# angela000/DQNFlappyBird

Measured on NVIDIA B200. Metric: env frames/sec (step+render+preproc), higher is better.
Workload: dtype u8

## Files before the change

dqnflappybird_b200/csrc/fb_common.cuh:

```cuda
#pragma once
#include <cuda_runtime.h>
#include <stdint.h>
#include <string>

#include "../../include/flappy_b200.h"

void fb_set_error(const std::string &msg);

#define FB_CUDA_OK(expr)                                                                      \
    do {                                                                                      \
        cudaError_t _e = (expr);                                                              \
        if (_e != cudaSuccess) {                                                              \
            fb_set_error(std::string(#expr) + ": " + cudaGetErrorString(_e));                 \
            return FB_ERR_CUDA;                                                               \
        }                                                                                     \
    } while (0)

#define FB_REQUIRE(cond, msg)                                                                 \
    do {                                                                                      \
        if (!(cond)) { fb_set_error(std::string(msg)); return FB_ERR_INVALID; }               \
    } while (0)

constexpr int kScreenW = 288, kScreenH = 512;
constexpr int kBirdW = 34, kBirdH = 24;
constexpr int kPipeW = 52, kPipeH = 320;
constexpr int kBaseW = 336, kBaseH = 112;
constexpr int kPlayerX = 57;
constexpr int kInitY = 244;
constexpr int kBaseYDraw = 404;
constexpr int kGroundY = 380;
constexpr int kBaseShift = kBaseW - kScreenW;
constexpr int kGapSize = 100;
constexpr int kMaxY = 379;

constexpr int kObs = FB_OBS;
constexpr int kBaseJ = 63;
constexpr int kBirdRows = 9;

struct __align__(16) EnvState {
    int16_t y;
    int8_t vel;
    uint8_t pidx;
    uint8_t loop;
    uint8_t phase;
    int8_t basex;
    uint8_t npipes;
    int16_t px[3];
    uint8_t gap[3];
    uint8_t pad0;
    int16_t pad1;
    int32_t score;
    uint32_t draws;
    uint32_t pad2;
};
static_assert(sizeof(EnvState) == 32, "EnvState must be 32 bytes");

struct ObsTables {
    unsigned long long pipeObs[54][5][8];
    unsigned char birdObs[3][kMaxY + 1][kBirdRows + 3];
    unsigned char birdJ0[kMaxY + 1 + 4];
    short sx[kObs];
};

static_assert(sizeof(ObsTables) % 16 == 0, "ObsTables is copied with 16-byte loads");

struct HitTables {
    unsigned long long birdRow[3][kBirdH];
    unsigned long long pipeRowLo[kPipeH];
    unsigned long long pipeRowUp[kPipeH];
};
static_assert(sizeof(HitTables) % 16 == 0, "HitTables is copied with 16-byte loads");

struct ExactTables {
    unsigned long long birdRow[3][kBirdH];
    unsigned long long pipeRowLo[kPipeH];
    unsigned long long pipeRowUp[kPipeH];
    uint32_t birdPix[3][kBirdW][kBirdH];
    uint32_t pipeLo[kPipeW][kPipeH];
    uint32_t pipeUp[kPipeW][kPipeH];
    uint32_t basePix[kBaseW][kBaseH];
    int sx[kObs], a0[kObs], a1[kObs];
    int sy[kObs], b0[kObs], b1[kObs];
};

struct FbTables {
    ObsTables *obs_dev;
    ExactTables *exact_dev;
    int device;
    bool loaded;
};
const FbTables &fb_tables();
const ObsTables *fb_host_obs_tables();
const ExactTables *fb_host_exact_tables();

__host__ __device__ inline void philox4x32_10(uint32_t c0, uint32_t c1, uint32_t c2, uint32_t c3, uint32_t k0,
                                              uint32_t k1, uint32_t out[4]) {
#pragma unroll
    for (int r = 0; r < 10; r++) {
#ifdef __CUDA_ARCH__
        uint32_t h0 = __umulhi(0xD2511F53u, c0), l0 = 0xD2511F53u * c0;
        uint32_t h1 = __umulhi(0xCD9E8D57u, c2), l1 = 0xCD9E8D57u * c2;
#else
        uint64_t p0 = (uint64_t)0xD2511F53u * c0, p1 = (uint64_t)0xCD9E8D57u * c2;
        uint32_t h0 = (uint32_t)(p0 >> 32), l0 = (uint32_t)p0, h1 = (uint32_t)(p1 >> 32), l1 = (uint32_t)p1;
#endif
        uint32_t n0 = h1 ^ c1 ^ k0, n2 = h0 ^ c3 ^ k1;
        c0 = n0; c1 = l1; c2 = n2; c3 = l0;
        k0 += 0x9E3779B9u; k1 += 0xBB67AE85u;
    }
    out[0] = c0; out[1] = c1; out[2] = c2; out[3] = c3;
}

__host__ __device__ inline uint32_t stream_word(uint64_t seed, uint32_t purpose, uint64_t env, uint32_t n) {
    uint32_t o[4];
    philox4x32_10(n >> 2, purpose, (uint32_t)env, (uint32_t)(env >> 32), (uint32_t)seed, (uint32_t)(seed >> 32), o);
    return o[n & 3];
}

__host__ __device__ inline int obs_pixel_gt1(uint32_t p00, uint32_t p01, uint32_t p10, uint32_t p11, int a0, int a1,
                                             int b0, int b1) {
    int v[3];
#pragma unroll
    for (int c = 0; c < 3; c++) {
        int s = 8 * c;
        int h0 = (int)((p00 >> s) & 255) * b0 + (int)((p01 >> s) & 255) * b1;
        int h1 = (int)((p10 >> s) & 255) * b0 + (int)((p11 >> s) & 255) * b1;
        v[c] = (((a0 * (h0 >> 4)) >> 16) + ((a1 * (h1 >> 4)) >> 16) + 2) >> 2;
    }
    int g = (3735 * v[0] + 19235 * v[1] + 9798 * v[2] + (1 << 14)) >> 15;
    return g > 1;
}
```

dqnflappybird_b200/csrc/fb_debug.cu:

```cuda
#include <stddef.h>
#include <string.h>

#include "fb_env_logic.cuh"

extern "C" int fb_debug_host_step(int32_t *state16, int action, const uint8_t *gaps, int gaps_len, uint64_t seed,
                                  uint64_t env_id, float *reward, uint8_t *terminal, int32_t *score) {
    const ExactTables *ex = fb_host_exact_tables();
    if (!ex) { fb_set_error("fb_debug_host_step: load the assets first"); return FB_ERR_ASSETS; }
    FB_REQUIRE(state16 && reward && terminal && score, "fb_debug_host_step: NULL argument");
    if (action != 0 && action != 1) { fb_set_error("Multiple input actions!"); return FB_ERR_ACTION; }
    EnvState s;
    memset(&s, 0, sizeof(s));
    if (!ints_to_state(state16, s)) { fb_set_error("fb_debug_host_step: state outside the reachable range"); return FB_ERR_STATE; }
    GapSource g{gaps, gaps_len, seed, env_id};
    env_step(s, action, g, ex, *reward, *terminal, *score);
    state_to_ints(s, state16);
    return FB_OK;
}

extern "C" int fb_debug_host_reset(int32_t *state16, const uint8_t *gaps, int gaps_len, uint64_t seed, uint64_t env_id) {
    FB_REQUIRE(state16 != nullptr, "fb_debug_host_reset: NULL argument");
    EnvState s;
    memset(&s, 0, sizeof(s));
    GapSource g{gaps, gaps_len, seed, env_id};
    env_reset(s, g);
    state_to_ints(s, state16);
    return FB_OK;
}

extern "C" int fb_debug_host_obs(const int32_t *state16, int mode, uint8_t *out) {
    const ObsTables *T = fb_host_obs_tables();
    const ExactTables *ex = fb_host_exact_tables();
    if (!T || !ex) { fb_set_error("fb_debug_host_obs: load the assets first"); return FB_ERR_ASSETS; }
    EnvState s;
    memset(&s, 0, sizeof(s));
    if (!ints_to_state(state16, s)) { fb_set_error("fb_debug_host_obs: state outside the reachable range"); return FB_ERR_STATE; }
    DrawList d = make_draw_list(s);
    if (mode == 1) {
        for (int i = 0; i < kObs; i++)
            for (int j = 0; j < kObs; j++) out[i * kObs + j] = exact_obs_bit(ex, d, s.basex, true, i, j) ? 255 : 0;
        return FB_OK;
    }
    const int j0 = T->birdJ0[d.y];
    for (int i = 0; i < kObs; i++) {
        unsigned long long m = obs_row_mask(*T, d, i);
        int r = i - 16;
        if ((d.np_mixed & 16) && r >= 0 && r < kBirdRows) {
            unsigned byte = 0;
            for (int b = 0; b < 8; b++)
                if (j0 + b < kBaseJ && exact_obs_bit(ex, d, 0, false, i, j0 + b)) byte |= 1u << b;
            m = obs_row_fix(m, byte, j0);
        }
        for (int j = 0; j < kObs; j++) out[i * kObs + j] = (j >= 64 || ((m >> j) & 1)) ? 255 : 0;
    }
    return FB_OK;
}

extern "C" int fb_debug_host_mixed(const int32_t *state16) {
    EnvState s;
    memset(&s, 0, sizeof(s));
    if (!ints_to_state(state16, s)) return -1;
    return (make_draw_list(s).np_mixed & 16) ? 1 : 0;
}

extern "C" int fb_debug_step_sampling_layout(int32_t *out, int capacity) {
    const int32_t v[] = {(int32_t)sizeof(fb_step_sampling),
                         (int32_t)offsetof(fb_step_sampling, replay), (int32_t)offsetof(fb_step_sampling, ring_dev),
                         (int32_t)offsetof(fb_step_sampling, act_dev), (int32_t)offsetof(fb_step_sampling, rew_dev),
                         (int32_t)offsetof(fb_step_sampling, term_dev), (int32_t)offsetof(fb_step_sampling, t),
                         (int32_t)offsetof(fb_step_sampling, batch), (int32_t)offsetof(fb_step_sampling, setsize),
                         (int32_t)offsetof(fb_step_sampling, seed), (int32_t)offsetof(fb_step_sampling, idx_out_dev),
                         (int32_t)offsetof(fb_step_sampling, frames_out_dev), (int32_t)offsetof(fb_step_sampling, act_out_dev),
                         (int32_t)offsetof(fb_step_sampling, rew_out_dev), (int32_t)offsetof(fb_step_sampling, term_out_dev),
                         (int32_t)offsetof(fb_step_sampling, env_out_dev), (int32_t)offsetof(fb_step_sampling, k_out_dev),
                         (int32_t)offsetof(fb_step_sampling, prioritized), (int32_t)offsetof(fb_step_sampling, per_mode),
                         (int32_t)offsetof(fb_step_sampling, beta), (int32_t)offsetof(fb_step_sampling, tree_idx_out_dev),
                         (int32_t)offsetof(fb_step_sampling, is_weights_out_dev), (int32_t)offsetof(fb_step_sampling, prio_out_dev),
                         (int32_t)offsetof(fb_step_sampling, is_weights_f32_out_dev)};
    const int n = (int)(sizeof(v) / sizeof(v[0]));
    FB_REQUIRE(out != nullptr && capacity >= n, "fb_debug_step_sampling_layout: buffer too small");
    for (int i = 0; i < n; i++) out[i] = v[i];
    return n;
}

__global__ void __launch_bounds__(256) write_probe_kernel(uint8_t *dst, int n_chunks, long long stride_bytes, int mode) {
    extern __shared__ __align__(128) uint8_t stage_all[];
    const int warp = threadIdx.x >> 5, lane = threadIdx.x & 31;
    uint8_t *stage = stage_all + warp * 6400;
    const long long W = (long long)gridDim.x * 8, w = (long long)blockIdx.x * 8 + warp;
    const int lo = (int)((long long)n_chunks * w / W), hi = (int)((long long)n_chunks * (w + 1) / W);
    if (mode == 1) {
        for (int i = lane; i < 400; i += 32) reinterpret_cast<uint4 *>(stage)[i] = make_uint4(i, lane, 0xFFFFFFFFu, 0);
        asm volatile("fence.proxy.async.shared::cta;" ::: "memory");
        __syncwarp();
    }
    for (int k = lo; k < hi; k++) {
        uint8_t *out = dst + (long long)k * stride_bytes;
        if (mode == 0) {
            const uint4 v = make_uint4(k, lane, 0xFFFFFFFFu, 0);
#pragma unroll
            for (int it = 0; it < 13; it++) { int c = lane + 32 * it; if (c < 400) __stcs(reinterpret_cast<uint4 *>(out) + c, v); }
        } else if (lane == 0) {
            asm volatile("cp.async.bulk.wait_group.read 0;" ::: "memory");
            asm volatile("cp.async.bulk.global.shared::cta.bulk_group [%0], [%1], 6400;" ::"l"(reinterpret_cast<uint64_t>(out)),
                         "r"((uint32_t)__cvta_generic_to_shared(stage)) : "memory");
            asm volatile("cp.async.bulk.commit_group;" ::: "memory");
        }
    }
    if (mode == 1 && lane == 0) asm volatile("cp.async.bulk.wait_group 0;" ::: "memory");
}

extern "C" int fb_debug_write_probe(uint8_t *dst_dev, int n_chunks, long long stride_bytes, int mode, int ctas, void *stream) {
    FB_REQUIRE(dst_dev && n_chunks > 0 && stride_bytes >= 6400 && (mode == 0 || mode == 1) && ctas > 0, "fb_debug_write_probe: bad argument");
    FB_CUDA_OK(cudaFuncSetAttribute(write_probe_kernel, cudaFuncAttributeMaxDynamicSharedMemorySize, 8 * 6400));
    write_probe_kernel<<<ctas, 256, 8 * 6400, (cudaStream_t)stream>>>(dst_dev, n_chunks, stride_bytes, mode);
    FB_CUDA_OK(cudaGetLastError());
    return FB_OK;
}
```

dqnflappybird_b200/csrc/fb_env.cu:

```cuda
#include <stdlib.h>

#include <new>

#include "fb_env_logic.cuh"

struct fb_env {
    int n;
    uint64_t seed, first_id;
    EnvState *state;
    const uint8_t *gaps;
    int gaps_len;
    int *err_flag;
    uint8_t *stage_act[2];
    float *stage_rew[2];
    uint8_t *stage_term[2];
    int32_t *stage_score[2];
    cudaStream_t s_in, s_out;
    cudaEvent_t ev_in[2], ev_step[2], ev_out[2];
    unsigned long long submitted, waited;
    int num_sms;
    int step_slots;
};

struct StepArgs {
    EnvState *state;
    int n;
    uint64_t seed, first_id;
    const uint8_t *gaps;
    int gaps_len;
    const uint8_t *actions;
    uint64_t act_seed;
    uint32_t first_step, flap_threshold;
    uint8_t *actions_out;
    uint8_t *ring;
    int ring_len, ring_slot;
    float *reward;
    uint8_t *terminal;
    int32_t *score;
    int n_steps;
    int draw_only;
    int *err_flag;
    const ObsTables *obs_tab;
    const ExactTables *ex;
};

__device__ __forceinline__ uint32_t expand4(uint32_t nib) {
    return ((nib * 0x00204081u) & 0x01010101u) * 255u;
}

struct RowConst { int sx[3], tab[3]; };

struct __align__(16) DrawWords {
    int px[3];
    int flags;
    int goff[3];
    int bird;
};
__device__ __forceinline__ DrawWords to_words(const ObsTables &T, const DrawList &d) {
    DrawWords w;
    const int np = d.np_mixed & 15;
#pragma unroll
    for (int k = 0; k < 3; k++) { w.px[k] = k < np ? (int)d.px[k] : 9999; w.goff[k] = (int)d.gap[k] * 8; }
    w.flags = ((d.np_mixed & 16) ? 1 : 0) | ((int)T.birdJ0[d.y] << 1) | ((int)d.y << 8) | ((int)d.pidx << 20) | (np << 24);
    w.bird = ((int)d.pidx * (kMaxY + 1) + (int)d.y) * (kBirdRows + 3);
    return w;
}

constexpr int kChunks = kObs * 5;

__device__ __forceinline__ void render_env(const ObsTables &T, const uint2 *lut8, const ExactTables *ex, const DrawWords w,
                                           const RowConst &rc, unsigned short *m16, unsigned long long *fixrows, uint8_t *out, int lane) {
    const int j0 = (w.flags >> 1) & 127;
    const unsigned char *pipe_bytes = reinterpret_cast<const unsigned char *>(&T.pipeObs[0][0][0]);
    const unsigned char *bird_bytes = reinterpret_cast<const unsigned char *>(&T.birdObs[0][0][0]) + w.bird;
    unsigned long long m[3];
#pragma unroll
    for (int it = 0; it < 3; it++) {
        unsigned long long v = 1ull << 63;
#pragma unroll
        for (int k = 0; k < 3; k++) {
            const unsigned c = (unsigned)(rc.sx[it] - w.px[k] + 1);
            if (c < 54u) v |= *reinterpret_cast<const unsigned long long *>(pipe_bytes + c * 320u + rc.tab[it] + w.goff[k]);
        }
        m[it] = v;
    }
    if (lane >= 16 && lane < 16 + kBirdRows) m[0] |= (unsigned long long)bird_bytes[lane - 16] << j0;
    if (w.flags & 1) {
        DrawList d;
        d.y = (int16_t)((w.flags >> 8) & 4095); d.pidx = (uint8_t)((w.flags >> 20) & 3); d.np_mixed = (uint8_t)(((w.flags >> 24) & 15) | 16);
#pragma unroll
        for (int k = 0; k < 3; k++) { d.px[k] = (int16_t)(w.px[k] == 9999 ? 0 : w.px[k]); d.gap[k] = (uint8_t)(w.goff[k] >> 3); d.pad[k] = 0; }
        if (lane >= 16 && lane < 16 + kBirdRows) fixrows[lane - 16] = m[0];
        __syncwarp();
#pragma unroll 1
        for (int q = 0; q < 3; q++) {
            int idx = q * 32 + lane, r = idx >> 3, j = j0 + (idx & 7);
            int bit = 0;
            if (r < kBirdRows && j < kBaseJ) bit = exact_obs_bit(ex, d, 0, false, 16 + r, j);
            unsigned bal = __ballot_sync(0xFFFFFFFFu, bit);
            int rr = 4 * q + lane;
            if (lane < 4 && rr < kBirdRows) fixrows[rr] = obs_row_fix(fixrows[rr], (bal >> (8 * lane)) & 0xFFu, j0);
        }
        __syncwarp();
        if (lane >= 16 && lane < 16 + kBirdRows) m[0] = fixrows[lane - 16];
    }
#pragma unroll
    for (int it = 0; it < 3; it++) {
        const int i = lane + 32 * it;
        if (i < kObs) {
            unsigned short *row = m16 + 5 * i;
            row[0] = (unsigned short)m[it]; row[1] = (unsigned short)(m[it] >> 16);
            row[2] = (unsigned short)(m[it] >> 32); row[3] = (unsigned short)(m[it] >> 48);
        }
    }
    __syncwarp();
    const unsigned short *mine = m16 + lane;
    uint4 *dst = reinterpret_cast<uint4 *>(out) + lane;
#pragma unroll
    for (int it = 0; it < 13; it++) {
        if (it < 12 || lane < kChunks - 32 * 12) {
            const uint32_t bits = mine[32 * it];
            const uint2 a = lut8[bits & 255u], b = lut8[bits >> 8];
            __stcs(dst + 32 * it, make_uint4(a.x, a.y, b.x, b.y));
        }
    }
    __syncwarp();
}

constexpr int kStepThreads = 256, kStepWarps = kStepThreads / 32;

__global__ void __launch_bounds__(kStepThreads, 4) env_step_kernel(const StepArgs a) {
    extern __shared__ __align__(16) unsigned char t_raw[];
    ObsTables &T = *reinterpret_cast<ObsTables *>(t_raw);
    __shared__ __align__(16) HitTables H;
    __shared__ DrawWords dw[kStepWarps][32];
    __shared__ __align__(16) unsigned short m16[kStepWarps][kChunks + 8];
    __shared__ unsigned long long fixrows[kStepWarps][kBirdRows + 1];
    __shared__ uint2 lut8[256];
    const int tid = threadIdx.x, warp = tid >> 5, lane = tid & 31;
    asm volatile("griddepcontrol.launch_dependents;");
    lut8[tid] = make_uint2(expand4(tid & 15u), expand4(tid >> 4));

    {
        const uint4 *srcH = reinterpret_cast<const uint4 *>(a.ex);
        uint4 *dstH = reinterpret_cast<uint4 *>(&H);
        for (int k = tid; k < (int)(sizeof(HitTables) / 16); k += kStepThreads) dstH[k] = __ldg(srcH + k);
    }
    if (a.ring) {
        const uint4 *src = reinterpret_cast<const uint4 *>(a.obs_tab);
        uint4 *dstT = reinterpret_cast<uint4 *>(&T);
        for (int k = tid; k < (int)(sizeof(ObsTables) / 16); k += kStepThreads) dstT[k] = __ldg(src + k);
    }
    __syncthreads();
    asm volatile("griddepcontrol.wait;" ::: "memory");

    RowConst rc;
#pragma unroll
    for (int it = 0; it < 3; it++) {
        const int i = min(lane + 32 * it, kObs - 1);
        rc.sx[it] = T.sx[i]; rc.tab[it] = (i - 5 * ((i * 205) >> 10)) * 64;
    }
    for (int i = lane; i < kObs; i += 32) m16[warp][5 * i + 4] = 0xFFFFu;
    __syncwarp();
    const long long W = (long long)gridDim.x * kStepWarps, w = (long long)blockIdx.x * kStepWarps + warp;
    const int lo = (int)((long long)a.n * w / W), hi = (int)((long long)a.n * (w + 1) / W);
    for (int base = lo; base < hi; base += 32) {
        const int e_mine = base + lane;
        const bool have = e_mine < hi;
        const int n_here = min(32, hi - base);
        EnvState s;
        GapSource gs;
        if (have) {
            const uint4 *sp = reinterpret_cast<const uint4 *>(a.state + e_mine);
            uint4 v0 = sp[0], v1 = sp[1];
            *reinterpret_cast<uint4 *>(&s) = v0;
            *(reinterpret_cast<uint4 *>(&s) + 1) = v1;
            gs.script = a.gaps ? a.gaps + (size_t)e_mine * a.gaps_len : nullptr;
            gs.script_len = a.gaps_len;
            gs.seed = a.seed; gs.env_id = a.first_id + (uint64_t)e_mine;
        }
        for (int step = 0; step < a.n_steps; step++) {
            if (have && a.draw_only) dw[warp][lane] = to_words(T, make_draw_list(s));
            if (have && !a.draw_only) {
                int act;
                const size_t o = (size_t)step * a.n + e_mine;
                if (a.actions) {
                    act = a.actions[o];
                    if (act > 1) { atomicOr(a.err_flag, 1); act = 0; }
                } else {
                    act = stream_word(a.act_seed, 1u, gs.env_id, a.first_step + (uint32_t)step) < a.flap_threshold ? 1 : 0;
                    if (a.actions_out) a.actions_out[o] = (uint8_t)act;
                }
                float rew; uint8_t term; int32_t sc;
                env_step(s, act, gs, &H, rew, term, sc);
                if (a.reward) a.reward[o] = rew;
                if (a.terminal) a.terminal[o] = term;
                if (a.score) a.score[o] = sc;
                if (a.ring) dw[warp][lane] = to_words(T, make_draw_list(s));
            }
            if (a.ring) {
                const int slot = (a.ring_slot + step) % a.ring_len;
                __syncwarp();
                for (int e = 0; e < n_here; e++) {
                    uint8_t *out = a.ring + ((size_t)(base + e) * a.ring_len + slot) * (size_t)FB_FRAME_BYTES;
                    render_env(T, lut8, a.ex, dw[warp][e], rc, m16[warp], fixrows[warp], out, lane);
                }
                __syncwarp();
            }
        }
        if (have) {
            uint4 *sp = reinterpret_cast<uint4 *>(a.state + e_mine);
            sp[0] = *reinterpret_cast<uint4 *>(&s);
            sp[1] = *(reinterpret_cast<uint4 *>(&s) + 1);
        }
    }
}


__global__ void env_reset_kernel(EnvState *state, int n, uint64_t seed, uint64_t first_id, const uint8_t *gaps, int gaps_len) {
    int e = blockIdx.x * blockDim.x + threadIdx.x;
    if (e >= n) return;
    EnvState s;
    memset(&s, 0, sizeof(s));
    GapSource gs{gaps ? gaps + (size_t)e * gaps_len : nullptr, gaps_len, seed, first_id + (uint64_t)e};
    env_reset(s, gs);
    state[e] = s;
}

__global__ void env_export_kernel(const EnvState *state, int n, int32_t *out) {
    int e = blockIdx.x * blockDim.x + threadIdx.x;
    if (e >= n) return;
    EnvState s = state[e];
    state_to_ints(s, out + (size_t)e * FB_STATE_INTS);
}

__global__ void env_import_kernel(EnvState *state, int n, const int32_t *in, int *err_flag) {
    int e = blockIdx.x * blockDim.x + threadIdx.x;
    if (e >= n) return;
    EnvState s;
    if (!ints_to_state(in + (size_t)e * FB_STATE_INTS, s)) { atomicOr(err_flag, 2); return; }
    state[e] = s;
}

__global__ void env_obs_exact_kernel(const EnvState *state, int n, const ExactTables *ex, uint8_t *obs) {
    int e = blockIdx.x;
    if (e >= n) return;
    __shared__ DrawList d;
    __shared__ int basex;
    if (threadIdx.x == 0) { EnvState s = state[e]; d = make_draw_list(s); basex = s.basex; }
    __syncthreads();
    for (int p = threadIdx.x; p < kObs * kObs; p += blockDim.x) {
        int i = p / kObs, j = p - i * kObs;
        obs[(size_t)e * FB_FRAME_BYTES + p] = exact_obs_bit(ex, d, basex, true, i, j) ? 255 : 0;
    }
}

__global__ void env_render_full_kernel(const EnvState *state, int first, int n, const ExactTables *ex, uint8_t *rgb) {
    int e = blockIdx.y;
    if (e >= n) return;
    __shared__ DrawList d;
    __shared__ int basex;
    if (threadIdx.x == 0) { EnvState s = state[first + e]; d = make_draw_list(s); basex = s.basex; }
    __syncthreads();
    int p = blockIdx.x * blockDim.x + threadIdx.x;
    if (p >= kScreenW * kScreenH) return;
    int X = p / kScreenH, Y = p - X * kScreenH;
    uint32_t c = scene_rgb(ex, d, basex, true, X, Y);
    uint8_t *o = rgb + ((size_t)e * kScreenW * kScreenH + p) * 3;
    o[0] = c & 255; o[1] = (c >> 8) & 255; o[2] = (c >> 16) & 255;
}


extern "C" int fb_env_create(int n_envs, uint64_t seed, uint64_t first_env_id, fb_env **out) {
    FB_REQUIRE(out != nullptr, "fb_env_create: out is NULL");
    FB_REQUIRE(n_envs > 0, "fb_env_create: n_envs must be positive");
    if (!fb_tables().loaded) { fb_set_error("fb_env_create: call fb_assets_load first"); return FB_ERR_ASSETS; }
    fb_env *e = new (std::nothrow) fb_env();
    FB_REQUIRE(e != nullptr, "fb_env_create: out of host memory");
    e->n = n_envs; e->seed = seed; e->first_id = first_env_id; e->gaps = nullptr; e->gaps_len = 0;
    int dev = 0;
    FB_CUDA_OK(cudaGetDevice(&dev));
    FB_CUDA_OK(cudaDeviceGetAttribute(&e->num_sms, cudaDevAttrMultiProcessorCount, dev));
    FB_CUDA_OK(cudaMalloc(&e->state, sizeof(EnvState) * (size_t)n_envs));
    FB_CUDA_OK(cudaMalloc(&e->err_flag, sizeof(int)));
    FB_CUDA_OK(cudaMemset(e->err_flag, 0, sizeof(int)));
    for (int k = 0; k < 2; k++) {
        FB_CUDA_OK(cudaMalloc(&e->stage_act[k], (size_t)n_envs));
        FB_CUDA_OK(cudaMalloc(&e->stage_rew[k], sizeof(float) * (size_t)n_envs));
        FB_CUDA_OK(cudaMalloc(&e->stage_term[k], (size_t)n_envs));
        FB_CUDA_OK(cudaMalloc(&e->stage_score[k], sizeof(int32_t) * (size_t)n_envs));
        FB_CUDA_OK(cudaEventCreateWithFlags(&e->ev_in[k], cudaEventDisableTiming));
        FB_CUDA_OK(cudaEventCreateWithFlags(&e->ev_step[k], cudaEventDisableTiming));
        FB_CUDA_OK(cudaEventCreateWithFlags(&e->ev_out[k], cudaEventDisableTiming));
    }
    FB_CUDA_OK(cudaStreamCreateWithFlags(&e->s_in, cudaStreamNonBlocking));
    FB_CUDA_OK(cudaStreamCreateWithFlags(&e->s_out, cudaStreamNonBlocking));
    e->submitted = e->waited = 0;
    e->step_slots = 0;
    *out = e;
    return fb_env_reset(e, nullptr);
}

extern "C" int fb_env_destroy(fb_env *e) {
    if (!e) return FB_OK;
    cudaFree(e->state); cudaFree(e->err_flag);
    for (int k = 0; k < 2; k++) {
        cudaFree(e->stage_act[k]); cudaFree(e->stage_rew[k]); cudaFree(e->stage_term[k]); cudaFree(e->stage_score[k]);
        if (e->ev_in[k]) cudaEventDestroy(e->ev_in[k]);
        if (e->ev_step[k]) cudaEventDestroy(e->ev_step[k]);
        if (e->ev_out[k]) cudaEventDestroy(e->ev_out[k]);
    }
    if (e->s_in) cudaStreamDestroy(e->s_in);
    if (e->s_out) cudaStreamDestroy(e->s_out);
    delete e;
    return FB_OK;
}

extern "C" int fb_env_num_envs(const fb_env *e) { return e ? e->n : 0; }

extern "C" int fb_env_set_gap_replay(fb_env *e, const uint8_t *gaps_dev, int per_env_len) {
    FB_REQUIRE(e != nullptr, "fb_env_set_gap_replay: env is NULL");
    FB_REQUIRE(gaps_dev == nullptr || per_env_len > 0, "fb_env_set_gap_replay: per_env_len must be positive");
    e->gaps = gaps_dev; e->gaps_len = gaps_dev ? per_env_len : 0;
    return FB_OK;
}

extern "C" int fb_env_reset(fb_env *e, void *stream) {
    FB_REQUIRE(e != nullptr, "fb_env_reset: env is NULL");
    env_reset_kernel<<<(e->n + 255) / 256, 256, 0, (cudaStream_t)stream>>>(e->state, e->n, e->seed, e->first_id, e->gaps, e->gaps_len);
    FB_CUDA_OK(cudaGetLastError());
    return FB_OK;
}

static int launch_step(fb_env *e, StepArgs &a, cudaStream_t st, bool early = true) {
    a.state = e->state; a.n = e->n; a.seed = e->seed; a.first_id = e->first_id;
    a.gaps = e->gaps; a.gaps_len = e->gaps_len; a.err_flag = e->err_flag;
    a.obs_tab = fb_tables().obs_dev; a.ex = fb_tables().exact_dev;
    if (e->step_slots == 0) {
        FB_CUDA_OK(cudaFuncSetAttribute(env_step_kernel, cudaFuncAttributeMaxDynamicSharedMemorySize, (int)sizeof(ObsTables)));
        int per_sm = 0;
        FB_CUDA_OK(cudaOccupancyMaxActiveBlocksPerMultiprocessor(&per_sm, env_step_kernel, kStepThreads, sizeof(ObsTables)));
        FB_REQUIRE(per_sm >= 1, "env_step_kernel does not fit an SM");
        e->step_slots = per_sm * e->num_sms;
    }
    static int oversub = 0;
    if (oversub == 0) { const char *v = getenv("FB_ENV_OVERSUB"); oversub = (v && v[0] >= '1' && v[0] <= '8') ? v[0] - '0' : 1; }
    long long warps = (long long)e->step_slots * kStepWarps * oversub;
    if (warps > e->n) warps = e->n;
    const int grid = (int)((warps + kStepWarps - 1) / kStepWarps);
    cudaLaunchConfig_t cfg{};
    cfg.gridDim = dim3(grid); cfg.blockDim = dim3(kStepThreads); cfg.dynamicSmemBytes = sizeof(ObsTables); cfg.stream = st;
    cudaLaunchAttribute at[1];
    at[0].id = cudaLaunchAttributeProgrammaticStreamSerialization;
    static int pdl = -1;
    if (pdl < 0) { const char *v = getenv("FB_ENV_PDL"); pdl = (v && v[0] == '0') ? 0 : 1; }
    at[0].val.programmaticStreamSerializationAllowed = pdl && early ? 1 : 0;
    cfg.attrs = at; cfg.numAttrs = 1;
    FB_CUDA_OK(cudaLaunchKernelEx(&cfg, env_step_kernel, (const StepArgs)a));
    return FB_OK;
}

static int check_ring(const fb_env *e, const uint8_t *ring, int ring_len, int ring_slot, int n_steps) {
    FB_REQUIRE(e != nullptr, "fb_env_step: env is NULL");
    FB_REQUIRE(n_steps > 0, "fb_env_step: n_steps must be positive");
    if (ring) {
        FB_REQUIRE(ring_len > 0 && ring_slot >= 0 && ring_slot < ring_len, "fb_env_step: ring_slot outside the ring");
        FB_REQUIRE((reinterpret_cast<uintptr_t>(ring) & 15) == 0, "fb_env_step: obs ring must be 16-byte aligned");
    }
    return FB_OK;
}

extern "C" int fb_env_step(fb_env *e, int n_steps, const uint8_t *actions_dev, uint8_t *obs_ring_dev, int ring_len,
                           int ring_slot, float *reward_dev, uint8_t *terminal_dev, int32_t *score_dev, void *stream) {
    int rc = check_ring(e, obs_ring_dev, ring_len, ring_slot, n_steps);
    if (rc) return rc;
    FB_REQUIRE(actions_dev != nullptr, "fb_env_step: actions_dev is NULL");
    StepArgs a{};
    a.actions = actions_dev; a.ring = obs_ring_dev; a.ring_len = ring_len; a.ring_slot = ring_slot;
    a.reward = reward_dev; a.terminal = terminal_dev; a.score = score_dev; a.n_steps = n_steps;
    return launch_step(e, a, (cudaStream_t)stream);
}

extern "C" int fb_env_draw(fb_env *e, uint8_t *obs_ring_dev, int ring_len, int ring_slot, void *stream) {
    int rc = check_ring(e, obs_ring_dev, ring_len, ring_slot, 1);
    if (rc) return rc;
    FB_REQUIRE(obs_ring_dev != nullptr, "fb_env_draw: obs_ring_dev is NULL");
    StepArgs a{};
    a.ring = obs_ring_dev; a.ring_len = ring_len; a.ring_slot = ring_slot; a.n_steps = 1; a.draw_only = 1;
    return launch_step(e, a, (cudaStream_t)stream);
}

extern "C" int fb_env_step_random(fb_env *e, int n_steps, uint64_t action_seed, uint32_t first_step, uint32_t flap_threshold,
                                  uint8_t *actions_out_dev, uint8_t *obs_ring_dev, int ring_len, int ring_slot,
                                  float *reward_dev, uint8_t *terminal_dev, int32_t *score_dev, void *stream) {
    int rc = check_ring(e, obs_ring_dev, ring_len, ring_slot, n_steps);
    if (rc) return rc;
    StepArgs a{};
    a.actions = nullptr; a.act_seed = action_seed; a.first_step = first_step; a.flap_threshold = flap_threshold;
    a.actions_out = actions_out_dev; a.ring = obs_ring_dev; a.ring_len = ring_len; a.ring_slot = ring_slot;
    a.reward = reward_dev; a.terminal = terminal_dev; a.score = score_dev; a.n_steps = n_steps;
    return launch_step(e, a, (cudaStream_t)stream);
}

static int host_submit(fb_env *e, const uint8_t *actions_host, uint8_t *obs_ring_dev, int ring_len, int ring_slot,
                       float *reward_host, uint8_t *terminal_host, int32_t *score_host, void *stream, bool split) {
    int rc = check_ring(e, obs_ring_dev, ring_len, ring_slot, 1);
    if (rc) return rc;
    FB_REQUIRE(actions_host != nullptr, "fb_env_step_host: actions_host is NULL");
    FB_REQUIRE(e->submitted - e->waited < 2, "fb_env_step_host_submit: two steps are already in flight; call fb_env_step_host_wait");
    cudaStream_t st = (cudaStream_t)stream;
    {
        const int n = e->n;
        int k = 0;
        unsigned long long bad = 0;
        for (; k + 8 <= n; k += 8) { unsigned long long w; memcpy(&w, actions_host + k, 8); bad |= w & 0xFEFEFEFEFEFEFEFEull; }
        for (; k < n; k++) bad |= (unsigned long long)(actions_host[k] & 0xFE);
        if (bad) { fb_set_error("Multiple input actions!"); return FB_ERR_ACTION; }
    }
    const int sl = (int)(e->submitted & 1);
    FB_CUDA_OK(cudaMemcpyAsync(e->stage_act[sl], actions_host, (size_t)e->n, cudaMemcpyHostToDevice, e->s_in));
    FB_CUDA_OK(cudaEventRecord(e->ev_in[sl], e->s_in));
    FB_CUDA_OK(cudaStreamWaitEvent(st, e->ev_in[sl], 0));
    StepArgs a{};
    a.actions = e->stage_act[sl]; a.ring = obs_ring_dev; a.ring_len = ring_len; a.ring_slot = ring_slot;
    a.reward = e->stage_rew[sl]; a.terminal = e->stage_term[sl]; a.score = e->stage_score[sl]; a.n_steps = 1;
    split = split && obs_ring_dev != nullptr;
    if (split) a.ring = nullptr;
    rc = launch_step(e, a, st, false);
    if (rc) return rc;
    FB_CUDA_OK(cudaEventRecord(e->ev_step[sl], st));
    if (split) {
        StepArgs d{};
        d.ring = obs_ring_dev; d.ring_len = ring_len; d.ring_slot = ring_slot; d.n_steps = 1; d.draw_only = 1;
        rc = launch_step(e, d, st);
        if (rc) return rc;
        FB_CUDA_OK(cudaEventRecord(e->ev_in[sl], st));
    }
    FB_CUDA_OK(cudaStreamWaitEvent(e->s_out, e->ev_step[sl], 0));
    if (reward_host) FB_CUDA_OK(cudaMemcpyAsync(reward_host, e->stage_rew[sl], sizeof(float) * (size_t)e->n, cudaMemcpyDeviceToHost, e->s_out));
    if (terminal_host) FB_CUDA_OK(cudaMemcpyAsync(terminal_host, e->stage_term[sl], (size_t)e->n, cudaMemcpyDeviceToHost, e->s_out));
    if (score_host) FB_CUDA_OK(cudaMemcpyAsync(score_host, e->stage_score[sl], sizeof(int32_t) * (size_t)e->n, cudaMemcpyDeviceToHost, e->s_out));
    if (split) FB_CUDA_OK(cudaStreamWaitEvent(e->s_out, e->ev_in[sl], 0));
    FB_CUDA_OK(cudaEventRecord(e->ev_out[sl], e->s_out));
    e->submitted++;
    return FB_OK;
}

extern "C" int fb_env_step_host_submit(fb_env *e, const uint8_t *actions_host, uint8_t *obs_ring_dev, int ring_len, int ring_slot,
                                       float *reward_host, uint8_t *terminal_host, int32_t *score_host, void *stream) {
    return host_submit(e, actions_host, obs_ring_dev, ring_len, ring_slot, reward_host, terminal_host, score_host, stream, false);
}

extern "C" int fb_env_step_host_wait(fb_env *e) {
    FB_REQUIRE(e != nullptr, "fb_env_step_host_wait: env is NULL");
    FB_REQUIRE(e->submitted > e->waited, "fb_env_step_host_wait: nothing in flight");
    FB_CUDA_OK(cudaEventSynchronize(e->ev_out[e->waited & 1]));
    e->waited++;
    return FB_OK;
}

extern "C" int fb_env_step_host(fb_env *e, const uint8_t *actions_host, uint8_t *obs_ring_dev, int ring_len, int ring_slot,
                                float *reward_host, uint8_t *terminal_host, int32_t *score_host, void *stream) {
    FB_REQUIRE(e != nullptr, "fb_env_step_host: env is NULL");
    while (e->submitted > e->waited) { int rc = fb_env_step_host_wait(e); if (rc) return rc; }
    int rc = host_submit(e, actions_host, obs_ring_dev, ring_len, ring_slot, reward_host, terminal_host, score_host, stream, e->n >= 8192);
    if (rc) return rc;
    return fb_env_step_host_wait(e);
}

extern "C" int fb_env_check(fb_env *e, void *stream) {
    FB_REQUIRE(e != nullptr, "fb_env_check: env is NULL");
    int flag = 0;
    FB_CUDA_OK(cudaMemcpyAsync(&flag, e->err_flag, sizeof(int), cudaMemcpyDeviceToHost, (cudaStream_t)stream));
    FB_CUDA_OK(cudaStreamSynchronize((cudaStream_t)stream));
    if (flag) {
        FB_CUDA_OK(cudaMemsetAsync(e->err_flag, 0, sizeof(int), (cudaStream_t)stream));
        if (flag & 1) { fb_set_error("Multiple input actions!"); return FB_ERR_ACTION; }
        fb_set_error("fb_env_import_state: state outside the reachable range");
        return FB_ERR_STATE;
    }
    return FB_OK;
}

extern "C" int fb_env_export_state(fb_env *e, int32_t *out_dev, void *stream) {
    FB_REQUIRE(e != nullptr && out_dev != nullptr, "fb_env_export_state: NULL argument");
    env_export_kernel<<<(e->n + 255) / 256, 256, 0, (cudaStream_t)stream>>>(e->state, e->n, out_dev);
    FB_CUDA_OK(cudaGetLastError());
    return FB_OK;
}

extern "C" int fb_env_import_state(fb_env *e, const int32_t *in_dev, void *stream) {
    FB_REQUIRE(e != nullptr && in_dev != nullptr, "fb_env_import_state: NULL argument");
    env_import_kernel<<<(e->n + 255) / 256, 256, 0, (cudaStream_t)stream>>>(e->state, e->n, in_dev, e->err_flag);
    FB_CUDA_OK(cudaGetLastError());
    return FB_OK;
}

extern "C" int fb_env_obs_exact(fb_env *e, uint8_t *obs_dev, void *stream) {
    FB_REQUIRE(e != nullptr && obs_dev != nullptr, "fb_env_obs_exact: NULL argument");
    env_obs_exact_kernel<<<e->n, 256, 0, (cudaStream_t)stream>>>(e->state, e->n, fb_tables().exact_dev, obs_dev);
    FB_CUDA_OK(cudaGetLastError());
    return FB_OK;
}

extern "C" int fb_render_full(fb_env *e, int first, int n, uint8_t *rgb_dev, void *stream) {
    FB_REQUIRE(e != nullptr && rgb_dev != nullptr, "fb_render_full: NULL argument");
    FB_REQUIRE(first >= 0 && n > 0 && first + n <= e->n, "fb_render_full: env range outside the handle");
    dim3 grid((kScreenW * kScreenH + 255) / 256, n);
    env_render_full_kernel<<<grid, 256, 0, (cudaStream_t)stream>>>(e->state, first, n, fb_tables().exact_dev, rgb_dev);
    FB_CUDA_OK(cudaGetLastError());
    return FB_OK;
}
```

dqnflappybird_b200/csrc/fb_env_logic.cuh:

```cuda
#pragma once
#include "fb_common.cuh"

#define FB_HD __host__ __device__ __forceinline__
#ifdef __CUDA_ARCH__
#define FB_LDG(p) __ldg(p)
#else
#define FB_LDG(p) (*(p))
#endif
FB_HD int fb_min(int a, int b) { return a < b ? a : b; }
FB_HD int fb_max(int a, int b) { return a > b ? a : b; }

struct __align__(16) DrawList {
    int16_t y;
    uint8_t pidx;
    uint8_t np_mixed;
    int16_t px[3];
    uint8_t gap[3];
    uint8_t pad[3];
};
static_assert(sizeof(DrawList) == 16, "DrawList must be 16 bytes");


struct GapSource {
    const uint8_t *script;
    int script_len;
    uint64_t seed, env_id;
};

FB_HD int draw_gap(EnvState &s, const GapSource &g) {
    if (g.script) {
        int v = g.script[s.draws % (uint32_t)g.script_len] & 7;
        s.draws++;
        return v;
    }
    for (;;) {
        uint32_t w = stream_word(g.seed, 0u, g.env_id, s.draws);
        s.draws++;
        if ((w >> 28) < 8u) return (int)(w >> 28);
    }
}

FB_HD void env_reset(EnvState &s, const GapSource &g) {
    s.score = 0; s.pidx = 0; s.loop = 0;
    s.y = kInitY; s.vel = 0; s.basex = 0;
    int g1 = draw_gap(s, g), g2 = draw_gap(s, g);
    s.px[0] = kScreenW; s.px[1] = kScreenW + kScreenW / 2; s.px[2] = 0;
    s.gap[0] = (uint8_t)g1; s.gap[1] = (uint8_t)g2; s.gap[2] = 0;
    s.npipes = 2;
}

template <class TB>
FB_HD bool hits_pipe(const EnvState &s, const TB *ex) {
    bool hit = false;
    for (int k = 0; k < s.npipes; k++) {
        int x = s.px[k];
        if (x >= kPlayerX + kBirdW || x + kPipeW <= kPlayerX) continue;
        int gapY = 100 + 10 * s.gap[k], y = s.y, sh = kPlayerX - x;
        int y_end = fb_min(y + kBirdH, gapY);
        for (int Y = y; Y < y_end; Y++) {
            unsigned long long b = ex->birdRow[s.pidx][Y - y], p = ex->pipeRowUp[Y - (gapY - kPipeH)];
            p = sh >= 0 ? p >> sh : p << (-sh);
            hit |= (b & p) != 0;
        }
        int ly = gapY + kGapSize;
        for (int Y = fb_max(y, ly); Y < y + kBirdH; Y++) {
            unsigned long long b = ex->birdRow[s.pidx][Y - y], p = ex->pipeRowLo[Y - ly];
            p = sh >= 0 ? p >> sh : p << (-sh);
            hit |= (b & p) != 0;
        }
    }
    return hit;
}

template <class TB>
FB_HD void env_step(EnvState &s, int action, const GapSource &g, const TB *ex,
                                         float &reward, uint8_t &terminal, int32_t &score_out) {
    reward = 0.1f;
    int vel = s.vel;
    if (action == 1) vel = -9;
    else if (vel < 10) vel += 1;
    s.vel = (int8_t)vel;
    int ny = s.y + vel;
    bool ground = ny >= kGroundY;
    if (!ground) s.y = (int16_t)fb_max(ny, 0);
    int loop1 = s.loop + 1;
    if (loop1 % 3 == 0) { s.pidx = (s.phase == 3) ? 1 : s.phase; s.phase = (s.phase + 1) & 3; }
    s.loop = (uint8_t)(loop1 == 30 ? 0 : loop1);
    s.basex = (int8_t)(-((100 - s.basex) % kBaseShift));
    for (int k = 0; k < 3; k++) if (k < s.npipes) s.px[k] -= 4;
    if (s.px[0] > 0 && s.px[0] < 5) {
        int gi = draw_gap(s, g);
        s.px[2] = kScreenW + 10; s.gap[2] = (uint8_t)gi; s.npipes = 3;
    }
    if (s.px[0] < -kPipeW) {
        s.px[0] = s.px[1]; s.px[1] = s.px[2]; s.gap[0] = s.gap[1]; s.gap[1] = s.gap[2];
        s.px[2] = 0; s.gap[2] = 0; s.npipes -= 1;
    }
    for (int k = 0; k < 3; k++)
        if (k < s.npipes && s.px[k] >= 45 && s.px[k] <= 48) { s.score += 1; reward = 3.0f; }
    bool crash = ground || hits_pipe(s, ex);
    score_out = s.score;
    terminal = crash ? 1 : 0;
    if (crash) { env_reset(s, g); reward = -3.0f; }
}

FB_HD DrawList make_draw_list(const EnvState &s) {
    DrawList d;
    d.y = s.y; d.pidx = s.pidx;
    bool mixed = false;
    for (int k = 0; k < 3; k++) {
        d.px[k] = s.px[k]; d.gap[k] = s.gap[k];
        if (k < s.npipes) {
            int x = s.px[k], gapY = 100 + 10 * s.gap[k];
            bool xo = x < kPlayerX + kBirdW + 1 && x + kPipeW > kPlayerX - 1;
            bool yo = gapY >= s.y || gapY + kGapSize < s.y + kBirdH + 1;
            mixed |= xo && yo;
        }
    }
    d.np_mixed = (uint8_t)(s.npipes | (mixed ? 16 : 0));
    d.pad[0] = d.pad[1] = d.pad[2] = 0;
    return d;
}


FB_HD uint32_t scene_rgb(const ExactTables *ex, const DrawList &d, int basex, bool with_base, int X, int Y) {
    int bx = X - kPlayerX, by = Y - d.y;
    if ((unsigned)bx < (unsigned)kBirdW && (unsigned)by < (unsigned)kBirdH) {
        uint32_t p = FB_LDG(&ex->birdPix[d.pidx][bx][by]);
        if (p >> 24) return p & 0xFFFFFFu;
    }
    if (with_base && Y >= kBaseYDraw) return FB_LDG(&ex->basePix[X - basex][Y - kBaseYDraw]) & 0xFFFFFFu;
    int np = d.np_mixed & 15;
    for (int k = 0; k < np; k++) {
        int c = X - d.px[k];
        if ((unsigned)c >= (unsigned)kPipeW) continue;
        int gapY = 100 + 10 * d.gap[k];
        uint32_t p = 0;
        if (Y < gapY) { int r = Y - (gapY - kPipeH); if (r >= 0) p = FB_LDG(&ex->pipeUp[c][r]); }
        else if (Y >= gapY + kGapSize) { int r = Y - (gapY + kGapSize); if (r < kPipeH) p = FB_LDG(&ex->pipeLo[c][r]); }
        if (p >> 24) return p & 0xFFFFFFu;
    }
    return 0u;
}

FB_HD int exact_obs_bit(const ExactTables *ex, const DrawList &d, int basex, bool with_base, int i, int j) {
    int sx = FB_LDG(&ex->sx[i]), sy = FB_LDG(&ex->sy[j]);
    uint32_t p00 = scene_rgb(ex, d, basex, with_base, sx, sy), p01 = scene_rgb(ex, d, basex, with_base, sx, sy + 1);
    uint32_t p10 = scene_rgb(ex, d, basex, with_base, sx + 1, sy), p11 = scene_rgb(ex, d, basex, with_base, sx + 1, sy + 1);
    return obs_pixel_gt1(p00, p01, p10, p11, FB_LDG(&ex->a0[i]), FB_LDG(&ex->a1[i]), FB_LDG(&ex->b0[j]), FB_LDG(&ex->b1[j]));
}


FB_HD unsigned long long obs_row_mask(const ObsTables &T, const DrawList &d, int i) {
    const int np = d.np_mixed & 15;
    int q5 = (i * 205) >> 10, ph5 = i - 5 * q5, sx = T.sx[i];
    unsigned long long m = 0;
#pragma unroll
    for (int k = 0; k < 3; k++) {
        unsigned c = (unsigned)(sx - d.px[k] + 1);
        if (k < np && c < 54u) m |= T.pipeObs[c][ph5][d.gap[k]];
    }
    unsigned r = (unsigned)(i - 16);
    if (r < (unsigned)kBirdRows) m |= (unsigned long long)T.birdObs[d.pidx][d.y][r] << T.birdJ0[d.y];
    return m | (1ull << 63);
}

FB_HD unsigned long long obs_row_fix(unsigned long long m, unsigned byte, int j0) {
    m = (m & ~(0xFFull << j0)) | ((unsigned long long)byte << j0);
    return m | (1ull << 63);
}

FB_HD void state_to_ints(const EnvState &s, int32_t *o) {
    o[0] = s.y; o[1] = s.vel; o[2] = s.pidx; o[3] = s.loop; o[4] = s.phase; o[5] = s.basex; o[6] = s.score; o[7] = s.npipes;
    for (int k = 0; k < 3; k++) { o[8 + k] = k < s.npipes ? s.px[k] : 0; o[11 + k] = k < s.npipes ? s.gap[k] : 0; }
    o[14] = (int32_t)s.draws; o[15] = 0;
}

FB_HD bool ints_to_state(const int32_t *o, EnvState &s) {
    s.y = (int16_t)o[0]; s.vel = (int8_t)o[1]; s.pidx = (uint8_t)o[2]; s.loop = (uint8_t)o[3]; s.phase = (uint8_t)o[4];
    s.basex = (int8_t)o[5]; s.npipes = (uint8_t)o[7];
    for (int k = 0; k < 3; k++) { s.px[k] = (int16_t)o[8 + k]; s.gap[k] = (uint8_t)o[11 + k]; }
    s.pad0 = 0; s.pad1 = 0; s.pad2 = 0;
    s.score = o[6]; s.draws = (uint32_t)o[14];
    bool ok = o[0] >= 0 && o[0] <= kMaxY && o[2] >= 0 && o[2] < 3 && o[3] >= 0 && o[3] < 30 && o[4] >= 0 && o[4] < 4 &&
              o[5] > -kBaseShift && o[5] <= 0 && o[7] >= 2 && o[7] <= 3 && o[1] >= -9 && o[1] <= 10;
    for (int k = 0; k < 3; k++) ok = ok && o[11 + k] >= 0 && o[11 + k] < 8 && o[8 + k] >= -60 && o[8 + k] <= 440;
    return ok;
}
```

Measured before the change: 836.8 million.

## Interleave env groups across CTAs and render with block-wide passes

The env step kernel now assigns groups of 8 consecutive envs round-robin across CTAs instead of giving each warp a contiguous range. Each thread steps one env and each warp then renders one env of the group per round, synchronising with __syncthreads instead of __syncwarp. Consecutive envs are written by neighbouring warps, and the grid is capped at resident slots with no oversubscription env var. Smaller changes make the stream_word index selection branch-free, unroll the pipe hit loop, and extend the debug write probe with sweep and plain-store modes. Block-wide barriers may add stalls compared with warp-local sync.

```diff
diff --git a/dqnflappybird_b200/csrc/fb_common.cuh b/dqnflappybird_b200/csrc/fb_common.cuh
--- a/dqnflappybird_b200/csrc/fb_common.cuh
+++ b/dqnflappybird_b200/csrc/fb_common.cuh
@@ -114,7 +114,8 @@
 __host__ __device__ inline uint32_t stream_word(uint64_t seed, uint32_t purpose, uint64_t env, uint32_t n) {
     uint32_t o[4];
     philox4x32_10(n >> 2, purpose, (uint32_t)env, (uint32_t)(env >> 32), (uint32_t)seed, (uint32_t)(seed >> 32), o);
-    return o[n & 3];
+    const uint32_t lo = (n & 1) ? o[1] : o[0], hi = (n & 1) ? o[3] : o[2];
+    return (n & 2) ? hi : lo;
 }
 
 __host__ __device__ inline int obs_pixel_gt1(uint32_t p00, uint32_t p01, uint32_t p10, uint32_t p11, int a0, int a1,
diff --git a/dqnflappybird_b200/csrc/fb_debug.cu b/dqnflappybird_b200/csrc/fb_debug.cu
--- a/dqnflappybird_b200/csrc/fb_debug.cu
+++ b/dqnflappybird_b200/csrc/fb_debug.cu
@@ -83,23 +83,33 @@
     return n;
 }
 
-__global__ void __launch_bounds__(256) write_probe_kernel(uint8_t *dst, int n_chunks, long long stride_bytes, int mode) {
+enum { kProbeBulk = 1, kProbeSweep = 2, kProbeDefault = 4, kProbeNoStage = 8 };
+
+__global__ void __launch_bounds__(256, 8) write_probe_kernel(uint8_t *dst, int n_chunks, long long stride_bytes, int mode) {
     extern __shared__ __align__(128) uint8_t stage_all[];
     const int warp = threadIdx.x >> 5, lane = threadIdx.x & 31;
     uint8_t *stage = stage_all + warp * 6400;
     const long long W = (long long)gridDim.x * 8, w = (long long)blockIdx.x * 8 + warp;
-    const int lo = (int)((long long)n_chunks * w / W), hi = (int)((long long)n_chunks * (w + 1) / W);
-    if (mode == 1) {
+    const bool bulk = mode & kProbeBulk, sweep = mode & kProbeSweep, dflt = mode & kProbeDefault;
+    long long lo = (long long)n_chunks * w / W, hi = (long long)n_chunks * (w + 1) / W, step = 1;
+    if (sweep) { lo = w; hi = n_chunks; step = W; }
+    if (bulk) {
         for (int i = lane; i < 400; i += 32) reinterpret_cast<uint4 *>(stage)[i] = make_uint4(i, lane, 0xFFFFFFFFu, 0);
         asm volatile("fence.proxy.async.shared::cta;" ::: "memory");
         __syncwarp();
     }
-    for (int k = lo; k < hi; k++) {
-        uint8_t *out = dst + (long long)k * stride_bytes;
-        if (mode == 0) {
-            const uint4 v = make_uint4(k, lane, 0xFFFFFFFFu, 0);
+    for (long long k = lo; k < hi; k += step) {
+        uint8_t *out = dst + k * stride_bytes;
+        if (!bulk) {
+            const uint4 v = make_uint4((unsigned)k, lane, 0xFFFFFFFFu, 0);
+            uint4 *o = reinterpret_cast<uint4 *>(out) + lane;
+            if (dflt) {
 #pragma unroll
-            for (int it = 0; it < 13; it++) { int c = lane + 32 * it; if (c < 400) __stcs(reinterpret_cast<uint4 *>(out) + c, v); }
+                for (int it = 0; it < 13; it++) if (lane + 32 * it < 400) o[32 * it] = v;
+            } else {
+#pragma unroll
+                for (int it = 0; it < 13; it++) if (lane + 32 * it < 400) __stcs(o + 32 * it, v);
+            }
         } else if (lane == 0) {
             asm volatile("cp.async.bulk.wait_group.read 0;" ::: "memory");
             asm volatile("cp.async.bulk.global.shared::cta.bulk_group [%0], [%1], 6400;" ::"l"(reinterpret_cast<uint64_t>(out)),
@@ -107,13 +117,15 @@
             asm volatile("cp.async.bulk.commit_group;" ::: "memory");
         }
     }
-    if (mode == 1 && lane == 0) asm volatile("cp.async.bulk.wait_group 0;" ::: "memory");
+    if (bulk && lane == 0) asm volatile("cp.async.bulk.wait_group 0;" ::: "memory");
 }
 
 extern "C" int fb_debug_write_probe(uint8_t *dst_dev, int n_chunks, long long stride_bytes, int mode, int ctas, void *stream) {
-    FB_REQUIRE(dst_dev && n_chunks > 0 && stride_bytes >= 6400 && (mode == 0 || mode == 1) && ctas > 0, "fb_debug_write_probe: bad argument");
+    FB_REQUIRE(dst_dev && n_chunks > 0 && stride_bytes >= 6400 && mode >= 0 && mode < 16 && ctas > 0, "fb_debug_write_probe: bad argument");
+    FB_REQUIRE(!((mode & kProbeBulk) && (mode & kProbeNoStage)), "fb_debug_write_probe: the bulk path needs its staging frames");
+    const int smem = (mode & kProbeNoStage) ? 0 : 8 * 6400;
     FB_CUDA_OK(cudaFuncSetAttribute(write_probe_kernel, cudaFuncAttributeMaxDynamicSharedMemorySize, 8 * 6400));
-    write_probe_kernel<<<ctas, 256, 8 * 6400, (cudaStream_t)stream>>>(dst_dev, n_chunks, stride_bytes, mode);
+    write_probe_kernel<<<ctas, 256, smem, (cudaStream_t)stream>>>(dst_dev, n_chunks, stride_bytes, mode);
     FB_CUDA_OK(cudaGetLastError());
     return FB_OK;
 }
diff --git a/dqnflappybird_b200/csrc/fb_env.cu b/dqnflappybird_b200/csrc/fb_env.cu
--- a/dqnflappybird_b200/csrc/fb_env.cu
+++ b/dqnflappybird_b200/csrc/fb_env.cu
@@ -127,17 +127,20 @@
     __syncwarp();
 }
 
-constexpr int kStepThreads = 256, kStepWarps = kStepThreads / 32;
+constexpr int kStepThreads = 256, kStepWarps = kStepThreads / 32, kGroupEnvs = kStepWarps;
 
 __global__ void __launch_bounds__(kStepThreads, 4) env_step_kernel(const StepArgs a) {
     extern __shared__ __align__(16) unsigned char t_raw[];
     ObsTables &T = *reinterpret_cast<ObsTables *>(t_raw);
     __shared__ __align__(16) HitTables H;
-    __shared__ DrawWords dw[kStepWarps][32];
+    __shared__ DrawWords dw[kStepThreads];
     __shared__ __align__(16) unsigned short m16[kStepWarps][kChunks + 8];
     __shared__ unsigned long long fixrows[kStepWarps][kBirdRows + 1];
     __shared__ uint2 lut8[256];
     const int tid = threadIdx.x, warp = tid >> 5, lane = tid & 31;
+    const int C = gridDim.x, c = blockIdx.x;
+    const int rounds = ((a.n + kGroupEnvs - 1) / kGroupEnvs - c + C - 1) / C;
+    const int rl = tid / kGroupEnvs, gk = tid % kGroupEnvs;
     asm volatile("griddepcontrol.launch_dependents;");
     lut8[tid] = make_uint2(expand4(tid & 15u), expand4(tid >> 4));
 
@@ -162,12 +165,11 @@
     }
     for (int i = lane; i < kObs; i += 32) m16[warp][5 * i + 4] = 0xFFFFu;
     __syncwarp();
-    const long long W = (long long)gridDim.x * kStepWarps, w = (long long)blockIdx.x * kStepWarps + warp;
-    const int lo = (int)((long long)a.n * w / W), hi = (int)((long long)a.n * (w + 1) / W);
-    for (int base = lo; base < hi; base += 32) {
-        const int e_mine = base + lane;
-        const bool have = e_mine < hi;
-        const int n_here = min(32, hi - base);
+    constexpr int kPassRounds = kStepThreads / kGroupEnvs;
+    for (int pass = 0; pass < rounds; pass += kPassRounds) {
+        const int e_mine = ((pass + rl) * C + c) * kGroupEnvs + gk;
+        const bool have = pass + rl < rounds && e_mine < a.n;
+        const int rounds_here = min(kPassRounds, rounds - pass);
         EnvState s;
         GapSource gs;
         if (have) {
@@ -180,7 +182,7 @@
             gs.seed = a.seed; gs.env_id = a.first_id + (uint64_t)e_mine;
         }
         for (int step = 0; step < a.n_steps; step++) {
-            if (have && a.draw_only) dw[warp][lane] = to_words(T, make_draw_list(s));
+            if (have && a.draw_only) dw[tid] = to_words(T, make_draw_list(s));
             if (have && !a.draw_only) {
                 int act;
                 const size_t o = (size_t)step * a.n + e_mine;
@@ -196,16 +198,18 @@
                 if (a.reward) a.reward[o] = rew;
                 if (a.terminal) a.terminal[o] = term;
                 if (a.score) a.score[o] = sc;
-                if (a.ring) dw[warp][lane] = to_words(T, make_draw_list(s));
+                if (a.ring) dw[tid] = to_words(T, make_draw_list(s));
             }
             if (a.ring) {
                 const int slot = (a.ring_slot + step) % a.ring_len;
-                __syncwarp();
-                for (int e = 0; e < n_here; e++) {
-                    uint8_t *out = a.ring + ((size_t)(base + e) * a.ring_len + slot) * (size_t)FB_FRAME_BYTES;
-                    render_env(T, lut8, a.ex, dw[warp][e], rc, m16[warp], fixrows[warp], out, lane);
+                __syncthreads();
+                for (int q = 0; q < rounds_here; q++) {
+                    const int e = ((pass + q) * C + c) * kGroupEnvs + warp;
+                    if (e >= a.n) break;
+                    uint8_t *out = a.ring + ((size_t)e * a.ring_len + slot) * (size_t)FB_FRAME_BYTES;
+                    render_env(T, lut8, a.ex, dw[q * kStepWarps + warp], rc, m16[warp], fixrows[warp], out, lane);
                 }
-                __syncwarp();
+                __syncthreads();
             }
         }
         if (have) {
@@ -343,11 +347,8 @@
         FB_REQUIRE(per_sm >= 1, "env_step_kernel does not fit an SM");
         e->step_slots = per_sm * e->num_sms;
     }
-    static int oversub = 0;
-    if (oversub == 0) { const char *v = getenv("FB_ENV_OVERSUB"); oversub = (v && v[0] >= '1' && v[0] <= '8') ? v[0] - '0' : 1; }
-    long long warps = (long long)e->step_slots * kStepWarps * oversub;
-    if (warps > e->n) warps = e->n;
-    const int grid = (int)((warps + kStepWarps - 1) / kStepWarps);
+    const int groups = (e->n + kGroupEnvs - 1) / kGroupEnvs;
+    const int grid = groups < e->step_slots ? groups : e->step_slots;
     cudaLaunchConfig_t cfg{};
     cfg.gridDim = dim3(grid); cfg.blockDim = dim3(kStepThreads); cfg.dynamicSmemBytes = sizeof(ObsTables); cfg.stream = st;
     cudaLaunchAttribute at[1];
diff --git a/dqnflappybird_b200/csrc/fb_env_logic.cuh b/dqnflappybird_b200/csrc/fb_env_logic.cuh
--- a/dqnflappybird_b200/csrc/fb_env_logic.cuh
+++ b/dqnflappybird_b200/csrc/fb_env_logic.cuh
@@ -52,7 +52,9 @@
 template <class TB>
 FB_HD bool hits_pipe(const EnvState &s, const TB *ex) {
     bool hit = false;
-    for (int k = 0; k < s.npipes; k++) {
+#pragma unroll
+    for (int k = 0; k < 3; k++) {
+        if (k >= s.npipes) continue;
         int x = s.px[k];
         if (x >= kPlayerX + kBirdW || x + kPipeW <= kPlayerX) continue;
         int gapY = 100 + 10 * s.gap[k], y = s.y, sh = kPlayerX - x;
```

After: 906.2 million, median of 6. 1.08x the previous value.
